# NorESMhub/BLOM

Measured on AMD Instinct MI355X. Metric: simulated-days/sec, higher is better.
Workload: dtype f64; 1 GPU; channel 208x512x53 as 1 tile(s) of 208x512x53 along i, 1 tile per GPU, isopyc_bulkml/remap/geopotential/uc/enscon, ntr=3 (TKE, length-scale slot, ideal age: the reference default build), baclin=900s batrop=18s lstep=50; config 2's step (phy/mod_blom_step.F90:96-253: init_fluxes, tmsmt1, cmnfld2, difest_isobml [the whole routine: diffusivities estimated every step (NorESM defaults incl. rhsctp; the; physics=full, forcing=default, spinup_steps=0

## Files before the change

### blom_amd/csrc/api.hip

```cpp
#include "../../include/blomgpu.h"
#include "blomgpu_internal.h"
#include "pow_libm.h"
#include "sin_libm.h"
#include "atan2_libm.h"
#include <algorithm>
#include <cstring>
#include <string_view>

static thread_local std::string g_err;

int ctx_fail(blomgpu_ctx *c, const std::string &msg) {
  if (c) c->err = msg;
  g_err = msg;
  return 1;
}

void ctx_drop_graphs(blomgpu_ctx *c) {
  for (auto &g : c->step_graph)
    if (g) { (void)hipGraphExecDestroy(g); g = nullptr; }
  c->steps_warm = 0;
}

void ctx_sync_view(blomgpu_ctx *c) {
  if (!c->dirty) return;
// ... 200 lines not shown
  {"mlrttp", O_STR, IN_C(mlrttp), 0},
  {"mommth", O_STR, IN_P(mommth), DIRTY, nullptr, nullptr, " mommth = ", {{"enscon", 0}, {"enecon", 1}, {"enedis", 2}}},
  {"pgfmth", O_STR, IN_P(pgfmth), DIRTY, nullptr, nullptr, " pgfmth = ", {{"geopotential", 0}, {"dynamic enthalpy", 1}}},
  {"advmth", O_STR, IN_P(advmth), DIRTY, nullptr, nullptr, " advmth = ", {{"remap", 0}, {"cppm", 1}}},
  {"bmcmth", O_STR, IN_P(bmcmth), DIRTY, nullptr, nullptr, " bmcmth = ", {{"uc", 0}, {"dluc", 1}}},
  {"eitmth", O_STR, IN_P(eitmth), DIRTY, nullptr, nullptr, " eitmth = ", {{"intdif", 1}, {"gm", 2}}},
  {"cppm_compatibility", O_STR, IN_C(cppm_compat), 0, nullptr, nullptr, " init_cppm: cppm_compatibility = ", {{"full", 1}, {"partial", 2}}},
  {"cppm_limiting", O_STR, IN_C(cppm_limiting), 0, nullptr, nullptr, " init_cppm: cppm_limiting = ", {{"monotonic", 1}, {"non_oscillatory", 2}}},
  {"mlrmth", O_STR, IN_C(mlrmth), 0, nullptr, nullptr, " init_eddtra: mlrmth = ", {{"none", 0}, {"fox08", 1}, {"bod23", 2}}},
  {"vcoord_type", O_STR, IN_P(vcoord_tag), DIRTY, nullptr, nullptr, " readnml_vcoord: vcoord_type = ",
   {{"isopyc_bulkml", 1}, {"cntiso_hybrid", 2}, {"plevel", 3}}},
  {"ale_reconstruction_method", O_STR, IN_C(ale_method), 0, nullptr, nullptr, " readnml_ale_regrid_remap: reconstruction_method = ",
   {{"plm", 101}, {"ppm", 102}, {"pqm", 103}}},
  {"ale_regrid_method", O_STR, IN_C(ale_regrid_method), 0, nullptr, nullptr, " readnml_ale_regrid_remap: regrid_method = ", {{"direct", 1}, {"nudge", 2}}},
  {"ale_density_limiting", O_STR, nullptr, 0, nullptr, nullptr, " readnml_ale_regrid_remap: density_limiting = ", {{"monotonic", 0}}},
  {"ale_tracer_limiting", O_STR, IN_C(ale_tracer_limiting), ALE_RESET, nullptr, nullptr, " readnml_ale_regrid_remap: tracer_limiting = ",
   {{"monotonic", 201}, {"non_oscillatory", 203}}},
  {"ale_velocity_limiting", O_STR, IN_C(ale_velocity_limiting), ALE_RESET, nullptr, nullptr, " readnml_ale_regrid_remap: velocity_limiting = ",
   {{"monotonic", 201}, {"non_oscillatory", 203}}},
};
static const Opt g_cesm_opts[] = {
  CB(smtfrc), CB(use_stream_relaxation), CI(nstep_in_cpl), CI(l1ci), CI(l2ci), CI(nstep_in_day), CI(nday_of_year), CI(cesm_single_sums),
};
static const Opt g_stepend_opts[] = {
  CB(step_time), CB(chkvar), CI(jwtype), {"chlopt", O_STR, IN_C(chlopt), 0},
  {"swamth", O_STR, IN_C(swamth), 0, nullptr, nullptr, " iniswa: swamth = ",
   {{"top-layer", SWA_TOP_LAYER}, {"jerlov", SWA_JERLOV}, {"chlorophyll_ma94", SWA_MA94}, {"chlorophyll_ohl03", SWA_OHL03}, {"spatial_frac_attlen", SWA_SPATIAL}}},
  {"sprfac", O_BOOL, IN_C(sprfac), 0, nullptr, [](blomgpu_ctx *c) { (void)stepend_set_sprfac(c); }},
  {"prfac", O_REAL, IN_C(prfac), READABLE},
};
static const Opt g_budget_opts[] = {
  CI(budget_step),
};
#undef IN_P
#undef IN_C
#undef PR
#undef PRR
#undef PI
#undef CR
#undef CI
#undef CB
#undef ONE_OR_TWO
#undef LMI
#undef RLX
static const Opt *find_opt(std::string_view name, unsigned kinds) {
  for (const Opt &o : g_opts)
    if (name == o.name && (kinds >> o.kind & 1)) return &o;
  for (const Opt &o : g_cesm_opts)
    if (name == o.name && (kinds >> o.kind & 1)) return &o;
  for (const Opt &o : g_stepend_opts)
    if (name == o.name && (kinds >> o.kind & 1)) return &o;
  for (const Opt &o : g_budget_opts)
    if (name == o.name && (kinds >> o.kind & 1)) return &o;
  return nullptr;
}
static int opt_lookup(blomgpu_ctx *c, const char *who, const char *name, unsigned kinds, const Opt **o) {
  if (!c || !name) return ctx_fail(c, std::string(who) + ": null argument");
  *o = find_opt(name, kinds);
  if (!*o || !((*o)->flags & KEEP_GRAPHS)) ctx_drop_graphs(c);
  return *o ? 0 : ctx_fail(c, std::string(who) + ": unknown option " + name);
}
static int set_number(blomgpu_ctx *c, const char *who, const char *name, unsigned kinds, double v) {
  const Opt *o;
  if (int rc = opt_lookup(c, who, name, kinds, &o)) return rc;
  if (o->kind == O_BOOL) v = v != 0;
  if (o->check)
    if (const char *refusal = o->check(v)) return ctx_fail(c, refusal);
  o->at(c).put(v);
  if (o->flags & DIRTY) c->dirty = true;
  if (o->after) o->after(c);
  return o->flags & ALE_RESET ? ale_reset(c) : 0;
}

template <class Launch>
static int libm_probe(blomgpu_ctx *c, int n, const double *a, const double *b, double *z, const char *who, Launch launch) {
  if (n <= 0) return 0;
  double *d = nullptr;
  HIPCHK(c, hipMalloc((void **)&d, sizeof(double) * 3 * (size_t)n));
  int rc = 0;
  if (hipMemcpyAsync(d, a, sizeof(double) * n, hipMemcpyHostToDevice, c->stream) != hipSuccess) rc = 1;
  if (b && hipMemcpyAsync(d + n, b, sizeof(double) * n, hipMemcpyHostToDevice, c->stream) != hipSuccess) rc = 1;
  launch(dim3((n + 255) / 256), d, d + n, d + 2 * (size_t)n);
  if (hipMemcpyAsync(z, d + 2 * (size_t)n, sizeof(double) * n, hipMemcpyDeviceToHost, c->stream) != hipSuccess) rc = 1;
  if (hipStreamSynchronize(c->stream) != hipSuccess) rc = 1;
  (void)hipFree(d);
// ... 137 lines not shown
  if (c->side) HIPCHK(c, hipStreamSynchronize(c->side));
  return 0;
}

int blomgpu_set_real(blomgpu_ctx *c, const char *name, double v) { return set_number(c, "blomgpu_set_real", name, 1u << O_REAL, v); }
int blomgpu_set_int(blomgpu_ctx *c, const char *name, int v) { return set_number(c, "blomgpu_set_int", name, 1u << O_INT | 1u << O_BOOL, v); }

int blomgpu_set_str(blomgpu_ctx *c, const char *name, const char *val) {
  const Opt *o = nullptr;
  const int rc = opt_lookup(c, "blomgpu_set_str", name, 1u << O_STR, &o);
  if (c) c->dirty = true;
  if (rc) return rc;
  if (!val) return ctx_fail(c, "blomgpu_set_str: null argument");
  const std::string v(val);
  if (!o->words[0].word) { *o->at(c).s = v; return 0; }
  for (const auto &w : o->words)
    if (w.word && v == w.word) {
      if (o->at) o->at(c).put(w.code);
      if (o->at && o->at(c).i == &c->swamth) c->swa_ready = false;
      return o->flags & ALE_RESET ? ale_reset(c) : 0;
    }
  return ctx_fail(c, o->refuse + v + " is unsupported!");
}

int blomgpu_get_real(blomgpu_ctx *c, const char *name, double *v) {
  const std::string s(name);
  if (const Opt *o = find_opt(s, 1u << O_REAL))
    if (o->flags & READABLE) { *v = *o->at(c).d; return 0; }
  if (s == "barotp_block_mode") { *v = bt_block_mode(c); return 0; }
  if (s == "barotp_shape") { *v = bt_shape_code(c); return 0; }
  if (s == "graph_steps") { *v = c->graph_steps; return 0; }
  if (s == "graph_failures") { *v = c->graph_failures; return 0; }
  if (s == "flux_diag_steps_skipped") { *v = (double)c->flux_diag_skipped; return 0; }
  if (s == "thermf_cesm_launches") { *v = (double)c->cesm_launches; return 0; }
  if (s == "thermf_ben02_launches") { *v = c->ben02_declared ? (double)c->cesm_launches : 0.; return 0; }
  if (c->step_time) {
    if (s == "xmi") { *v = c->xmi; return 0; }
    if (s == "nday_of_year") { *v = c->nday_of_year; return 0; }
    if (s.size() == 4 && s[0] == 'l' && s[1] >= '1' && s[1] <= '5' && s.compare(2, 2, "mi") == 0) { *v = c->lmi[s[1] - '1']; return 0; }
  }
  if (s == "sflxc") {
    if (!frc_declared(c)) return ctx_fail(c, "blomgpu_get_real: sflxc exists once blomgpu_inifrc_cesm has been called");
    double sum = 0.;
    HIPCHK(c, hipMemcpyAsync(&sum, c->cesm_sums, sizeof(double), hipMemcpyDeviceToHost, c->stream));
    HIPCHK(c, hipStreamSynchronize(c->stream));
    *v = sum / c->area;
    return 0;
  }
  if (s == "mxlayr_maxitr_entrain" || s == "mxlayr_maxitr_detrain") {
    *v = 0.;
    if (!c->err_dev) return 0;
    const int w = s == "mxlayr_maxitr_detrain" ? 5 : 6;
    int n = 0;
    HIPCHK(c, hipStreamSynchronize(c->stream));
    HIPCHK(c, hipMemcpy(&n, c->err_dev + w, sizeof(int), hipMemcpyDeviceToHost));
    HIPCHK(c, hipMemset(c->err_dev + w, 0, sizeof(int)));
    *v = n;
    return 0;
  }
  return ctx_fail(c, "blomgpu_get_real: unknown option " + s);
}

int blomgpu_option_name(int index, char *buf, int cap, int *kind) {
  if (index < 0 || index >= (int)(sizeof(g_opts) / sizeof(g_opts[0])) || !buf || cap < 2) return 1;
  snprintf(buf, cap, "%s", g_opts[index].name);
  if (kind) *kind = g_opts[index].kind;
// ... 432 lines not shown
    if (int rc = bud(1)) return rc;
    if (ale) {
      for (const StageId st : seq_ale) {
        if (c->tmsmt1_done_ahead && st == S_tmsmt1) { c->tmsmt1_done_ahead = false; continue; }
        if (c->eddtra_frozen && st == S_eddtra) continue;
        if (frc && st == S_pgforc)
          if (int rc = stage(S_sfcstr)) return rc;
        if (int rc = stage(st)) return rc;
        if (const int ncall = st == S_ale_regrid_remap ? 2 : st == S_diffus ? 3 : st == S_ale_vdiffm ? 4 : st == S_updtrc ? 5 : st == S_pbcor2 ? 6 : st == S_tmsmt2 ? 7 : 0)
          if (int rc = bud(ncall)) return rc;
        if (cesm && st == S_init_fluxes)
          if (int rc = stage(S_getfrc_cesm)) return rc;
        if (swa && st == S_init_fluxes)
          if (int rc = stage(S_updswa)) return rc;
        if (frc && st == S_momtum)
          if (int rc = stage(S_thermf)) return rc;
      }
    } else for (const StageId st : seq) {
      StageId run = c->live_slopes && st == S_halo_cmnfld2 ? S_cmnfld2 : st;
      if (c->full_physics && st == S_halo_difest) run = c->difest_live ? S_difest_isobml : S_difest_isobml_pre;
      if (c->full_physics && st == S_mxlayr_tail) {
        if (int rc = stage(S_thermf)) return rc;
        run = S_mxlayr;
      }
      if (c->eddtra_frozen && st == S_eddtra) continue;
      if (c->tmsmt1_done_ahead && st == S_tmsmt1) { c->tmsmt1_done_ahead = false; continue; }
      if (c->seq.fluxes_lean) {
        bool allowed = false;
        for (const StageId ok : {S_tmsmt1, S_halo_cmnfld2, S_cmnfld2, S_halo_difest, S_difest_isobml, S_difest_isobml_pre, S_eddtra, S_advect})
          allowed = allowed || run == ok;
        if (!allowed)
          return ctx_fail(c, std::string("blomgpu_step: stage ") + g_stages[run].name + " between the lean init_fluxes and advect: the flux arrays of level m are not zeroed (set lean_fluxes = 0)");
      }
      if ((c->seq.diapfl_mom_on_side && run != S_mxlayr) || (c->seq.updtrc_on_side && st == S_pbcor2)) {
        const int ev = c->seq.diapfl_mom_on_side ? 7 : 9;
        c->seq.diapfl_mom_on_side = c->seq.updtrc_on_side = false;
        if (ctx_side_done(c, ev) || ctx_side_join(c, ev)) return 1;
      }
      if (frc && st == S_pgforc)
        if (int rc = stage(S_sfcstr)) return rc;
      if (int rc = stage(run)) return rc;
      if (const int ncall = st == S_diffus ? 2 : st == S_convec ? 3 : st == S_diapfl ? 4 : st == S_updtrc ? 5 : st == S_pbcor2 ? 6 : st == S_tmsmt2 ? 7 : 0) {
        if (ncall == 5 && budget_on(c) && c->seq.updtrc_on_side) {
          c->seq.updtrc_on_side = false;
          if (ctx_side_done(c, 9) || ctx_side_join(c, 9)) return 1;
        }
        if (int rc = bud(ncall)) return rc;
      }
      if (cesm && st == S_init_fluxes)
        if (int rc = stage(S_getfrc_cesm)) return rc;
      if (swa && st == S_init_fluxes)
        if (int rc = stage(S_updswa)) return rc;
      if (st == S_halo_difest && c->seq.cmn_on_side) {
        c->seq.cmn_on_side = false;
        if (ctx_side_done(c, 4) || ctx_side_join(c, 4)) return 1;
      }
      static const StageId early_at[] = {S_halo_difest, S_eddtra, S_advect, S_pbcor1, S_diffus};
      if (st == early_at[c->mom_early_at < 0 || c->mom_early_at > 4 ? 0 : c->mom_early_at])
        if (int rc = st_momtum_early(c, m, n, mm, nn)) return rc;
    }
    leave.failed = false;
  }
  if (!ale && (c->cmnfld1 || c->full_physics))
    if (int rc = stage(S_cmnfld1)) return rc;
  if (dia_active(c))
    if (int rc = st_diaacc(ALL6)) return rc;
// ... 145 lines not shown
```

### blom_amd/csrc/blomgpu_internal.h

```cpp
#pragma once
#include <hip/hip_runtime.h>
#include <cstdint>
#include <string>
#include <unordered_map>
#include <vector>
#include "exp_libm.h"
#include "constants.h"
#include "workspace_slots.h"

#define NBDY 4

#ifdef BLOM_HOSTEMU
#define WAIT_VMCNT0() ((void)0)
#else
#define WAIT_VMCNT0() asm volatile("s_waitcnt vmcnt(0)" ::: "memory")
#endif

#define BLOM_REAL_FIELDS(X)                                                              \
                                                                          \
  X(u, 2 * K) X(v, 2 * K) X(dp, 2 * K) X(dpu, 2 * K) X(dpv, 2 * K) X(temp, 2 * K)        \
  X(saln, 2 * K) X(sigma, 2 * K) X(uflx, 2 * K) X(vflx, 2 * K) X(utflx, 2 * K)           \
  X(vtflx, 2 * K) X(usflx, 2 * K) X(vsflx, 2 * K)                                        \
  X(p, K + 1) X(pu, K + 1) X(pv, K + 1) X(phi, K + 1) X(cau, K) X(cav, K)                \
  X(ubflxs, 3) X(vbflxs, 3) X(ub, 2) X(vb, 2) X(pb, 2) X(pbu, 2) X(pbv, 2)               \
// ... 206 lines not shown
struct BtGlobal;
struct DiaState;
struct BudgetState;
struct TileTable {
  int npx = 0, npy = 0, itdm = 0, nranks = 0;
  std::vector<int> i0, ii;
  std::vector<int> j0, jj;
  std::vector<int> rank;
  void ew_neighbours(int px, int py, bool periodic, int *west, int *east) const;
  bool tensor_product() const;
};
const char *tiletable_build(int npx, int npy, int itdm, int jtdm, const int *i0_pe, const int *ii_pe, const int *j0_pe,
                            const int *jj_pe, TileTable *out);
struct Tiling {
  int npx = 1, npy = 1;
  int px = 0, py = 0;
  const TileTable *tab = nullptr;
  TileGroup *group = nullptr;
  RcclComm *rccl = nullptr;
  bool multi() const { return npx * npy > 1 || rccl != nullptr; }
};

struct StepState {
  bool in_sequence = false;
  bool defer_checks = false;
  bool remap_handed_over = false;
  bool pbcor1_handed_over = false;
  bool pbcor2_handed_over = false;
  bool pbcor2_dp_in_wk = false;
  bool fluxes_lean = false;
  bool fluxes_zeroed = false;
  bool mom_early_done = false;
  bool convec_col_ahead = false;
  bool cmn_on_side = false;
  bool diapfl_mom_on_side = false, updtrc_on_side = false;
  bool pscan_done_ahead = false;
};

struct BtShape { int ti, tj, pair_pref; bool persist, block; };
constexpr int BT_NSHAPES = 7;
constexpr BtShape kBtShapes[BT_NSHAPES] = {{32, 16, 4, false, false}, {32, 8, 2, false, false}, {16, 8, 1, false, false},
                                           {26, 16, 3, true, true},   {26, 15, 0, true, true},  {40, 16, 5, true, false},
                                           {40, 15, 0, true, false}};

struct blomgpu_ctx {
  std::string expcnf = "channel";
  bool csdiag = false;
  int cnsvdi = 0;
  int cppm_compat = 1;
  int cppm_limiting = 2;
  int ale_method = 102, ale_upper_bndr_ord = 6, ale_lower_bndr_ord = 4, ale_tracer_limiting = 203, ale_velocity_limiting = 203;
  bool ale_tracer_pc_upper = true, ale_tracer_pc_lower = false, ale_velocity_pc_upper = true, ale_velocity_pc_lower = false;
  bool ale_density_pc_upper = false, ale_density_pc_lower = false;
  int ale_regrid_method = 2, ale_k_range_plevel = 1;
  double ale_regrid_nudge_ts = 86400., ale_stab_fac_limit = .75, ale_dpvar_fac = .75, ale_smooth_diff_max = 50000.;
  int ale_dktzu = 4, ale_dktzl = 2;
  double ale_dpmin_interior = .1 * ONEM;
  int ndiff_rec_per_face = 0;
  int ndiff_surface_align = 1;
  double rm0 = 1.2, rm5 = 0., niwgf = 0., niwbf = .35, niwlf = .5;
  std::string mlrttp = "constant";
  double trxday = 0., srxday = 0., trxdpt = 1., srxdpt = 1., trxlim = 1.5, srxlim = .5, sref = 34.65, area = 0., xmi = 0.;
  int lmi[5] = {11, 12, 1, 2, 3};
  bool aptflx = false, apsflx = false, ditflx = false, disflx = false, srxbal = false;
  int ntda = 0;
  double swamxd = 200., brine_mlbase_frac = 0.;
// ... 15 lines not shown
  int check_period = 8;
  bool timing = false;
  int use_graph = 0;
  int overlap = 1;
  int phys_dag = 7;
  int mom_early_at = 0;
  int lean_fluxes = 1;
  int tmsmt_fold = 1;
  int tmsmt_ahead = 1;
  int remap_fold = 0;
  int remap_nfirst = 4;
  int halo_overlap = 1;
  int barotp_fused = 1;
  int barotp_tile = 0;
  int barotp_persist = 1;
  int barotp_block = 1;
  int barotp_overlap = 0;
  int barotp_rimbuf = 1;
  int barotp_arctic_persist = 1;
  int barotp_arctic_fused = 1;
  int arctic_strips = 0;
  int pgf_uv_pair = 0;
  int pgf_uv_ring = 7;
  int pgf_reuse = 0;
  int pgf_copy_fused = 1;
  int scan_reassoc = 0;
  int mom_aw_split = 0;
  int mom_force_aw = 0;
  int momtum_order = 0;
  int momtum_lds_pad = 0;
  int momtum_bs = 0;
  int momtum_chunks_a = 0, momtum_chunks_b = 0;
  int convec_nsingle = 2;
  int cmn_nslope_nb = 4;
  int diapfl_du = 8;
  int diffus_shfl = 0;
  int kprof_sel = 1;

  DevView h;
  DevView *d = nullptr;
  bool dirty = true;
  int device = 0;
  hipStream_t stream = nullptr;
  bool stream_borrowed = false;
  hipStream_t xstream = nullptr, halo_stream = nullptr;
  hipEvent_t ev_fork = nullptr, ev_join = nullptr;
  hipStream_t side = nullptr;
  hipEvent_t ev_side[10] = {};
  DevView hv[4];
  DevView *dv[4] = {nullptr, nullptr, nullptr, nullptr};
  double *wk_mom = nullptr, *p_alt = nullptr, *pu_alt = nullptr, *pv_alt = nullptr;
  hipStream_t side3 = nullptr;
  hipEvent_t ev_side3[2] = {nullptr, nullptr};
  int mom_aw_key = -1, mom_aw_n[2] = {0, 0};
  int *mom_aw_dev = nullptr;
  int nlev_real[NF_REAL];
  int nlev_int[NF_INT];
  std::unordered_map<std::string, int> real_ids, int_ids;
  std::unordered_map<std::string, KTimer> timers;
  Tiling tiling;
  BtGlobal *bt_global = nullptr;
  std::string err;
  int *err_dev = nullptr;
  StepState seq;
  bool tmsmt1_ahead = false, tmsmt1_done_ahead = false;
  bool flux_diag = true, keep_flux_diag = false;
  long long flux_diag_skipped = 0;
  hipGraphExec_t step_graph[2] = {nullptr, nullptr};
  int steps_done = 0;
  int steps_warm = 0;
  long long graph_steps = 0;
  int graph_failures = 0;
  bool cppm_ready = false;
  void *ale = nullptr;
  double *ale_plevel = nullptr;
  bool bt_restart = true;
  unsigned bt_epoch = 0;
  unsigned *bt_flags = nullptr;
  int bt_flags_words = 0;
  int num_cus = 0;
  int bt_blocks_per_cu[BT_NSHAPES][2] = {{-1, -1}, {-1, -1}, {-1, -1}, {-1, -1}, {-1, -1}, {-1, -1}, {-1, -1}};
  long long *bt_prof = nullptr;
  long long *kprof = nullptr;
  int kprof_words = 0;
  double *arc_strip = nullptr;
  size_t arc_cap = 0;
  double *xcsum_dev = nullptr;
  double *xcsum_buf = nullptr;
  double budget[5][7][2] = {};
  int budget_step = 0;
  BudgetState *bud = nullptr;
  DiaState *dia = nullptr;
  std::vector<double> dia_edges;
  std::vector<double> dia_sigdia;
  bool cesm_declared = false;
  int nflxdi[48] = {};
  long long cesm_launches = 0;
  double *cesm_sums = nullptr, *cesm_rows = nullptr;
  bool ben02_declared = false;
// ... 21 lines not shown
static inline bool flux_diag_on(const blomgpu_ctx *c) { return !c->seq.in_sequence || c->flux_diag; }

int  ctx_fail(blomgpu_ctx *c, const std::string &msg);
int  ctx_pack_masks(blomgpu_ctx *c);
void ctx_sync_view(blomgpu_ctx *c);
void ctx_drop_graphs(blomgpu_ctx *c);
#define HIPCHK(c, call)                                                                   \
  do {                                                                                    \
    hipError_t e_ = (call);                                                               \
    if (e_ != hipSuccess)                                                                 \
      return ctx_fail((c), std::string(#call) + ": " + hipGetErrorString(e_));            \
  } while (0)

struct TimeScope {
  blomgpu_ctx *c;
  hipEvent_t a = nullptr, b = nullptr;
  const char *what;
  hipStream_t st = nullptr;
  TimeScope(blomgpu_ctx *c_, const char *w, hipStream_t s = nullptr);
  ~TimeScope();
};

int st_init_fluxes(blomgpu_ctx *, int m, int n, int mm, int nn, int k1m, int k1n);
int st_tmsmt1(blomgpu_ctx *, int nn);
int st_tmsmt2(blomgpu_ctx *, int m, int mm, int nn, int k1m);
int st_initms(blomgpu_ctx *, int mm);
int st_advect(blomgpu_ctx *, int m, int n, int mm, int nn, int k1m, int k1n);
int st_pbcor1(blomgpu_ctx *, int m, int n, int mm, int nn, int k1m, int k1n);
int st_pbcor2(blomgpu_ctx *, int m, int n, int mm, int nn, int k1m, int k1n);
int st_diffus(blomgpu_ctx *, int m, int n, int mm, int nn, int k1m, int k1n);
int st_pgforc(blomgpu_ctx *, int m, int n, int mm, int nn, int k1m, int k1n);
int st_momtum(blomgpu_ctx *, int m, int n, int mm, int nn, int k1m, int k1n);
int st_momtum_fused_layers(blomgpu_ctx *, int m, int n, int mm, int nn, int part);
int st_momtum_early(blomgpu_ctx *, int m, int n, int mm, int nn);
int st_convec_column_ahead(blomgpu_ctx *, int n, int nn);
int st_diapfl(blomgpu_ctx *, int n, int nn, int k1n);
int st_convec(blomgpu_ctx *, int m, int n, int mm, int nn, int k1m, int k1n);
int st_updtrc(blomgpu_ctx *, int m, int n, int mm, int nn, int k1m, int k1n);
int st_xcsum(blomgpu_ctx *, const double *a, int itype, double *sum);
int st_xcsum_dev(blomgpu_ctx *, const double *a, int itype, int slot, double **sums_dev);
int st_thermf(blomgpu_ctx *, int m, int n, int mm, int nn, int k1m, int k1n);
int cesm_inifrc(blomgpu_ctx *);
int cesm_field(blomgpu_ctx *, int fid);
void cesm_free(blomgpu_ctx *);
static inline bool cesm_on(const blomgpu_ctx *c) { return c->cesm_declared && c->expcnf == "cesm"; }
int frc_alloc(blomgpu_ctx *, double **p, int nlev);
int frc_sum_buffers(blomgpu_ctx *);
int st_getfrc_cesm(blomgpu_ctx *);
int st_sfcstr_cesm(blomgpu_ctx *);
int st_thermf_cesm(blomgpu_ctx *, int m, int n, int mm, int nn, int k1m, int k1n);
static inline bool ben02_expcnf(const std::string &e) { return e == "ben02clim" || e == "ben02syn" || e == "single_column"; }
static inline bool ben02_on(const blomgpu_ctx *c) { return c->ben02_declared && ben02_expcnf(c->expcnf); }
static inline bool frc_declared(const blomgpu_ctx *c) { return c->cesm_declared || c->ben02_declared; }
int ben02_inifrc(blomgpu_ctx *);
int ben02_reset_tda(blomgpu_ctx *);
void ben02_free(blomgpu_ctx *);
int st_sfcstr_ben02(blomgpu_ctx *);
int st_thermf_ben02(blomgpu_ctx *, int m, int n, int mm, int nn, int k1m, int k1n);
enum { SWA_NONE = 0, SWA_TOP_LAYER, SWA_JERLOV, SWA_MA94, SWA_OHL03, SWA_SPATIAL };
static inline bool swa_chlorophyll(const blomgpu_ctx *c) { return c->swamth == SWA_MA94 || c->swamth == SWA_OHL03; }
int stepend_iniswa(blomgpu_ctx *);
int stepend_set_sprfac(blomgpu_ctx *);
int stepend_step_time(blomgpu_ctx *, int ns1);
int stepend_step_check(blomgpu_ctx *);
int stepend_check_errors(blomgpu_ctx *);
void stepend_free(blomgpu_ctx *);
// ... 190 lines not shown
```

### blom_amd/csrc/stage_convec.hip

```cpp
#include "blomgpu_internal.h"
#include "eos.h"
#include "diapfl_common.h"

#define MAXTR 64

__global__ __launch_bounds__(64) void k_convec_column(const DevView *__restrict__ Vp, int n, int nn, int *errflag) {
  const DevView &V = *Vp;
  THREAD_IJ_XCD(V);
  if (j < 1 || j > V.jj || i < 1 || i > V.ii || !V.m[I_ip][c]) return;
  const int kk = V.kk, ntr = V.ntr;
  const size_t np = V.nplane;
  gd_t ttem = V.f[F_temp] + c + (size_t)nn * np - np, ssal = V.f[F_saln] + c + (size_t)nn * np - np;
  gd_t delp = V.f[F_dp] + c + (size_t)nn * np - np, dens = V.f[F_sigma] + c + (size_t)nn * np - np;
  gcd_t densr = V.f[F_sigmar] + c - np;
  gd_t trc = V.f[F_trc] + c + (size_t)nn * np - np;
  const size_t ntl = (size_t)2 * kk * np;
#define TT(k) ttem[(size_t)(k) * np]
#define SS(k) ssal[(size_t)(k) * np]
#define DP(k) delp[(size_t)(k) * np]
#define DN(k) dens[(size_t)(k) * np]
#define DR(k) densr[(size_t)(k) * np]
#define TR(nt, k) trc[(size_t)(nt) * ntl + (size_t)(k) * np]
  double tdps, sdps, dps, ttmp, stmp, dtmp, q = 0.;

// ... 367 lines not shown
  switch (c->convec_nsingle) {
    case -1: hipLaunchKernelGGL(k_convec_velocity_flat, plane_grid(c->h, 2, 64), dim3(64), 0, c->stream, c->d, nn); break;
    case 0: hipLaunchKernelGGL(k_convec_velocity<0>, plane_grid(c->h, 2, 64), dim3(64), 0, c->stream, c->d, nn); break;
    case 1: hipLaunchKernelGGL(k_convec_velocity<1>, plane_grid(c->h, 2, 64), dim3(64), 0, c->stream, c->d, nn); break;
    case 2: hipLaunchKernelGGL(k_convec_velocity<2>, plane_grid(c->h, 2, 64), dim3(64), 0, c->stream, c->d, nn); break;
    case 3: hipLaunchKernelGGL(k_convec_velocity<3>, plane_grid(c->h, 2, 64), dim3(64), 0, c->stream, c->d, nn); break;
    default: hipLaunchKernelGGL(k_convec_velocity<1000>, plane_grid(c->h, 2, 64), dim3(64), 0, c->stream, c->d, nn); break;
  }
  HIPCHK(c, hipGetLastError());
  return 0;
}

int st_convec_column_ahead(blomgpu_ctx *c, int n, int nn) {
  const DevView &h = c->h;
  c->seq.convec_col_ahead = false;
  if (h.ntr > MAXTR || h.P.vcoord_tag != 1) return 0;
  if (int rc = ctx_err_words(c)) return rc;
  if (int rc = ctx_side_fork(c, 2)) return rc;
  hipLaunchKernelGGL(k_convec_column, plane_grid(h, 1, 64), dim3(64), 0, c->side, c->d, n, nn, c->err_dev + 3);
  HIPCHK(c, hipGetLastError());
  if (int rc = ctx_side_done(c, 3)) return rc;
  c->seq.convec_col_ahead = true;
  return 0;
}

int st_convec(blomgpu_ctx *c, int m, int n, int mm, int nn, int k1m, int k1n) {
  (void)m; (void)mm; (void)k1m; (void)k1n;
  const DevView &h = c->h;
  if (h.ntr > MAXTR) return ctx_fail(c, "convec: too many tracers for the device kernels");
  if (h.P.vcoord_tag != 1) return ctx_fail(c, "convec is only called for isopyc_bulkml (phy/mod_blom_step.F90:172-176)");
  if (int rc = ctx_err_words(c)) return rc;
  {
    TimeScope ts(c, "convec");
    if (c->seq.convec_col_ahead) {
      c->seq.convec_col_ahead = false;
      if (int rc = ctx_side_join(c, 3)) return rc;
    } else
      hipLaunchKernelGGL(k_convec_column, plane_grid(h, 1, 64), dim3(64), 0, c->stream, c->d, n, nn, c->err_dev + 3);
    if (int rc = st_xctilr(c, h.f[F_p], 1, h.kk + 1, 1, 1, 1)) return rc;
    if (int rc = st_convec_velocity(c, nn)) return rc;
    hipLaunchKernelGGL(k_convec_dpudpv, plane_grid(h, h.kk), dim3(256), 0, c->stream, c->d, nn);
  }
  HIPCHK(c, hipGetLastError());
  return 0;
}
```

### blom_amd/csrc/stage_momtum.hip

```cpp
#include "blomgpu_internal.h"

#include "momtum_common.h"


__global__ void k_mom_pupv(const DevView *__restrict__ Vp, int off, int lo, int hi, int ring) {
  const DevView &V = *Vp;
  THREAD_IJ_XCD(V);
  if (j < lo || j > V.jj + hi || i < lo || i > V.ii + hi) return;
  if (ring && j >= 1 && j <= V.jj && i >= 1 && i <= V.ii) return;
  const size_t np = V.nplane;
  if (V.m[I_iu][c]) column_scan(V.f[F_pu][c], V.f[F_dpu] + (size_t)off * np + c, V.f[F_pu] + c, np, V.kk);
  if (V.m[I_iv][c]) column_scan(V.f[F_pv][c], V.f[F_dpv] + (size_t)off * np + c, V.f[F_pv] + c, np, V.kk);
}

__global__ void k_mom_pscan(const DevView *__restrict__ Vp, int off, int lo, int hi, int ring) {
  const DevView &V = *Vp;
  THREAD_IJ_XCD(V);
  if (j < lo || j > V.jj + hi || i < lo || i > V.ii + hi || !V.m[I_ip][c]) return;
  if (ring && j >= 1 && j <= V.jj && i >= 1 && i <= V.ii) return;
  const size_t np = V.nplane;
  column_scan(V.f[F_p][c], V.f[F_dp] + (size_t)off * np + c, V.f[F_p] + c, np, V.kk);
}

__global__ void k_mom_drag(const DevView *__restrict__ Vp, int n, int nn) {
// ... 43 lines not shown
    q[c + np] = V.f[F_vbflxs_p][c + om] * tsfac / (V.f[F_pbv][c + om] * sx);
    q[c + 3 * np] = V.f[F_vbflxs_p][c + on] * tsfac / (V.f[F_pbv][c + on] * sx);
  }
}

int st_mom_pupv(blomgpu_ctx *c, int off, int lo, int hi) {
  hipLaunchKernelGGL(k_mom_pupv, plane_grid(c->h, 1, 64), dim3(64), 0, c->stream, c->d, off, lo, hi, 0);
  HIPCHK(c, hipGetLastError());
  return 0;
}

static int momtum_visc_chain(blomgpu_ctx *c, int m, int n, int mm, int nn) {
  const DevView &h = c->h;
  hipLaunchKernelGGL(k_mom_pupv, plane_grid(h, 1, 64), dim3(64), 0, c->stream, ctx_view(c, VIEW_MOM_A), mm, -1, 2, 0);
  hipLaunchKernelGGL(k_mom_qplanes, plane_grid(h, 1, 256), dim3(256), 0, c->stream, ctx_view(c, VIEW_MOM_A), m, n);
  return st_momtum_fused_layers(c, m, n, mm, nn, 1);
}

int st_momtum_early(blomgpu_ctx *c, int m, int n, int mm, int nn) {
  c->seq.mom_early_done = false;
  if (!ctx_overlap_on(c) || c->tiling.multi()) return 0;
  if (int rc = st_xctilr(c, c->h.f[F_difwgt], 1, 1, 2, 2, 1)) return rc;
  if (int rc = ctx_side_fork(c, 0)) return rc;
  hipStream_t main = c->stream;
  c->stream = c->side;
  const int rc = momtum_visc_chain(c, m, n, mm, nn);
  c->stream = main;
  if (rc) return rc;
  if (int rc2 = ctx_side_done(c, 1)) return rc2;
  c->seq.mom_early_done = true;
  return 0;
}

int st_momtum(blomgpu_ctx *c, int m, int n, int mm, int nn, int k1m, int k1n) {
  (void)k1m; (void)k1n;
  const DevView &h = c->h;
  const dim3 gcol = plane_grid(h, 1, 64), b64(64);
  if (ctx_overlap_on(c) && !c->tiling.multi())
    if (int rc = st_convec_column_ahead(c, n, nn)) return rc;
  TimeScope ts(c, "momtum");
  hipLaunchKernelGGL(k_mom_pscan, gcol, b64, 0, c->stream, ctx_view(c, VIEW_MOM_B), mm, -1, 2, 0);
  hipLaunchKernelGGL(k_mom_pscan, gcol, b64, 0, c->stream, c->d, mm, -1, 2, c->seq.in_sequence && h.P.vcoord_tag == 1 ? 1 : 0);
  hipLaunchKernelGGL(k_mom_pupv, gcol, b64, 0, c->stream, c->d, mm, -1, 2, 1);
  hipLaunchKernelGGL(k_mom_drag, gcol, b64, 0, c->stream, ctx_view(c, VIEW_MOM_B), n, nn);
  if (c->seq.mom_early_done) {
    c->seq.mom_early_done = false;
    if (int rc = ctx_side_join(c, 1)) return rc;
  } else {
    if (int rc = st_xctilr(c, h.f[F_difwgt], 1, 1, 2, 2, 1)) return rc;
    if (int rc = momtum_visc_chain(c, m, n, mm, nn)) return rc;
  }
  return st_momtum_fused_layers(c, m, n, mm, nn, 2);
}
```

### blom_amd/csrc/stage_momtum_fused.hip

```cpp
#include "momtum_common.h"
#include <type_traits>

#define WK2V(w) ((gcd_t) * (double *const volatile CONST_AS *)&Vp->wk2d + (size_t)(w) * np)

#define GLOBAL_AS BLOM_GAS
#define GF(V, id) ((gcd_t)(V).f[id])

__device__ inline void march_item(int kk, int jj, int nchunk_, int nstrip, int &k, int &ja, int &jb, int &strip, const int *list = nullptr) {
  const bool chunk_major = nchunk_ < 0;
  const int nchunk = chunk_major ? -nchunk_ : nchunk_;
  const unsigned nitem = gridDim.x, lin = blockIdx.x;
  const unsigned xq = lin & 7u, sq = lin >> 3, q = nitem >> 3, rr = nitem & 7u;
  unsigned item = xq * q + (xq < rr ? xq : rr) + sq;
  if (list) {
    const int e = list[item / kk];
    k = item % kk;
    strip = e % nstrip;
    const int ch = e / nstrip, rows = (jj + nchunk - 1) / nchunk;
    ja = 1 + ch * rows;
    jb = ja + rows - 1 < jj ? ja + rows - 1 : jj;
    return;
  }
  strip = item % nstrip;
  item /= nstrip;
// ... 618 lines not shown
        un = fmax2(-umax, fmin2(umax, un + ub)) - ub;
        un_[(size_t)k * np] = un;
        uabove = un;
        tot = tot + un * dn;
      }
    }
  }
  tot = tot / (isv ? V.f[F_pbv_p] : V.f[F_pbu_p])[c];
  double pacc = (isv ? V.f[F_pv] : V.f[F_pu])[c];
  gd_t pun = (isv ? V.f[F_pv] : V.f[F_pu]) + c;
  for (int k0 = 0; k0 < kk; k0 += COLUMN_U) {
    double a[COLUMN_U], b[COLUMN_U], d[COLUMN_U], e[COLUMN_U], f[COLUMN_U];
#pragma unroll
    for (int u = 0; u < COLUMN_U; u++) {
      const size_t o = (size_t)(k0 + u < kk ? k0 + u : kk - 1) * np;
      a[u] = dpum[o]; b[u] = dpun[o]; d[u] = un_[o]; e[u] = sm[o]; f[u] = dpuold[o];
    }
#pragma unroll
    for (int u = 0; u < COLUMN_U; u++) {
      const int k = k0 + u;
      if (k < kk) {
        const double dn = b[u];
        const double un = d[u] - tot;
        un_[(size_t)k * np] = un;
        um[(size_t)k * np] = (e[u] + un * wuv2 * dn) / (wuv1 * a[u] + ONEMM + wuv2 * (f[u] + dn));
        pacc = pacc + dn;
        pun[(size_t)(k + 1) * np] = pacc;
      }
    }
  }
  (isv ? V.f[F_vtotn] : V.f[F_utotn])[c] = tot * (1. / V.P.delt1);
}

template <int BS>
__global__ __launch_bounds__(64) void k_mom_classify(const DevView *__restrict__ Vp, int nchunk, int nstrip, int *flags) {
  const DevView &V = *Vp;
  const int l = threadIdx.x, ni = V.ni, ii = V.ii, jj = V.jj;
  const int e = blockIdx.x, strip = e % nstrip, ch = e / nstrip;
  const int rows = (jj + nchunk - 1) / nchunk, ja = 1 + ch * rows, jb = ja + rows - 1 < jj ? ja + rows - 1 : jj;
  constexpr int HL = 4, HR = 4, OW = BS - HL - HR;
  const int ox0 = NBDY + strip * OW;
  bool all = ja <= jb && ox0 <= ii + NBDY - 1;
  for (int l0 = 0; l0 < BS; l0 += 64) {
    const int x = ox0 - HL + l0 + l;
    const int xl = x < 2 ? 2 : (x > ni - 3 ? ni - 3 : x);
    for (int r = ja - 6; r <= jb + 4; r++) {
      const int rc = r < -2 ? -2 : (r > jj + 3 ? jj + 3 : r);
      if ((V.m[I_mpack][xl + ni * (rc + NBDY - 1)] & 15) != 15) all = false;
    }
  }
  all = WAVE_ALL(all);
  if (l == 0) flags[e] = all ? 1 : 0;
}

static int mom_aw_lists(blomgpu_ctx *c, int BS, int nca, int nsa, const int **la_, int *na, const int **lb_, int *nb) {
  const int key = BS * 100000 + nca * 100 + nsa;
  if (c->mom_aw_key != key) {
    hipStreamCaptureStatus cs = hipStreamCaptureStatusNone;
    if (hipStreamIsCapturing(c->stream, &cs) != hipSuccess || cs != hipStreamCaptureStatusNone) return 1;
    if (c->mom_aw_dev) { (void)hipFree(c->mom_aw_dev); c->mom_aw_dev = nullptr; }
    const int n = nca * nsa;
    int *flags = nullptr;
    HIPCHK(c, hipMalloc((void **)&flags, sizeof(int) * n));
    ctx_sync_view(c);
    if (BS == 64) hipLaunchKernelGGL(k_mom_classify<64>, dim3(n), dim3(64), 0, c->stream, c->d, nca, nsa, flags);
    else if (BS == 128) hipLaunchKernelGGL(k_mom_classify<128>, dim3(n), dim3(64), 0, c->stream, c->d, nca, nsa, flags);
    else hipLaunchKernelGGL(k_mom_classify<256>, dim3(n), dim3(64), 0, c->stream, c->d, nca, nsa, flags);
    std::vector<int> hf(n), lists;
    HIPCHK(c, hipMemcpyAsync(hf.data(), flags, sizeof(int) * n, hipMemcpyDeviceToHost, c->stream));
    HIPCHK(c, hipStreamSynchronize(c->stream));
    (void)hipFree(flags);
    for (int e = 0; e < n; e++) if (hf[e]) lists.push_back(e);
    c->mom_aw_n[0] = (int)lists.size();
    for (int e = 0; e < n; e++) if (!hf[e]) lists.push_back(e);
    c->mom_aw_n[1] = n - c->mom_aw_n[0];
    HIPCHK(c, hipMalloc((void **)&c->mom_aw_dev, sizeof(int) * (n > 0 ? n : 1)));
    HIPCHK(c, hipMemcpy(c->mom_aw_dev, lists.data(), sizeof(int) * n, hipMemcpyHostToDevice));
    c->mom_aw_key = key;
  }
  *la_ = c->mom_aw_dev; *na = c->mom_aw_n[0];
  *lb_ = c->mom_aw_dev + c->mom_aw_n[0]; *nb = c->mom_aw_n[1];
  return 0;
}

template <int BS>
static void launch_marches(blomgpu_ctx *c, int m, int n, int mm, int nn, int nca, int ncb, int part) {
  const DevView &h = c->h;
  const int nsa = (h.ii + (BS - 8) - 1) / (BS - 8), nsb = (h.ii + (BS - 4) - 1) / (BS - 4);
  const size_t la = sizeof(double) * 37 * (BS + 4) + c->momtum_lds_pad, lb = sizeof(double) * (h.P.mommth == 2 ? 35 : 21) * (BS + 4) + c->momtum_lds_pad;
  (void)hipFuncSetAttribute((const void *)k_mom_visc_march<BS, 2>, hipFuncAttributeMaxDynamicSharedMemorySize, (int)la);
  (void)hipFuncSetAttribute((const void *)k_mom_cor_march<BS, true>, hipFuncAttributeMaxDynamicSharedMemorySize, (int)lb);
  (void)hipFuncSetAttribute((const void *)k_mom_cor_march<BS, false>, hipFuncAttributeMaxDynamicSharedMemorySize, (int)lb);
  if (part != 2) {
    TimeScope tk(c, "k_mom_visc_march");
    (void)hipFuncSetAttribute((const void *)k_mom_visc_march<BS, 1>, hipFuncAttributeMaxDynamicSharedMemorySize, (int)la);
    const int *l_aw = nullptr, *l_mx = nullptr;
    int n_aw = 0, n_mx = 0;
    const bool split = c->mom_aw_split && h.P.allwet && !c->mom_force_aw && !c->momtum_order && mom_aw_lists(c, BS, nca, nsa, &l_aw, &n_aw, &l_mx, &n_mx) == 0;
    if (c->mom_force_aw)
      hipLaunchKernelGGL((k_mom_visc_march<BS, 1>), dim3(h.kk * nca * nsa), dim3(BS), la, c->stream, ctx_view(c, VIEW_MOM_A), m, n, mm, nn, c->momtum_order ? nca : -nca, nsa, (const int *)nullptr);
    else if (split) {
      const bool third = n_aw && n_mx && c->mom_aw_split == 2;
      if (third) {
        if (!c->side3) {
          if (hipStreamCreateWithFlags(&c->side3, hipStreamNonBlocking) != hipSuccess) c->side3 = nullptr;
          for (auto &e : c->ev_side3) if (hipEventCreateWithFlags(&e, hipEventDisableTiming) != hipSuccess) e = nullptr;
        }
      }
      if (third && c->side3 && c->ev_side3[0] && c->ev_side3[1]) {
        (void)hipEventRecord(c->ev_side3[0], c->stream);
        (void)hipStreamWaitEvent(c->side3, c->ev_side3[0], 0);
        hipLaunchKernelGGL((k_mom_visc_march<BS, 2>), dim3(h.kk * n_mx), dim3(BS), la, c->side3, ctx_view(c, VIEW_MOM_A), m, n, mm, nn, -nca, nsa, l_mx);
        hipLaunchKernelGGL((k_mom_visc_march<BS, 1>), dim3(h.kk * n_aw), dim3(BS), la, c->stream, ctx_view(c, VIEW_MOM_A), m, n, mm, nn, -nca, nsa, l_aw);
        (void)hipEventRecord(c->ev_side3[1], c->side3);
        (void)hipStreamWaitEvent(c->stream, c->ev_side3[1], 0);
      } else {
        if (n_mx) hipLaunchKernelGGL((k_mom_visc_march<BS, 2>), dim3(h.kk * n_mx), dim3(BS), la, c->stream, ctx_view(c, VIEW_MOM_A), m, n, mm, nn, -nca, nsa, l_mx);
        if (n_aw) hipLaunchKernelGGL((k_mom_visc_march<BS, 1>), dim3(h.kk * n_aw), dim3(BS), la, c->stream, ctx_view(c, VIEW_MOM_A), m, n, mm, nn, -nca, nsa, l_aw);
      }
    } else
      hipLaunchKernelGGL((k_mom_visc_march<BS, 2>), dim3(h.kk * nca * nsa), dim3(BS), la, c->stream, ctx_view(c, VIEW_MOM_A), m, n, mm, nn, c->momtum_order ? nca : -nca, nsa, (const int *)nullptr);
  }
  if (part == 1) return;
  TimeScope tk(c, "k_mom_cor_march");
  if (h.P.mommth == 2)
    hipLaunchKernelGGL((k_mom_cor_march<BS, true>), dim3(h.kk * ncb * nsb), dim3(BS), lb, c->stream, ctx_view(c, VIEW_MOM_B), m, n, mm, nn, c->momtum_order ? ncb : -ncb, nsb);
  else
    hipLaunchKernelGGL((k_mom_cor_march<BS, false>), dim3(h.kk * ncb * nsb), dim3(BS), lb, c->stream, ctx_view(c, VIEW_MOM_B), m, n, mm, nn, c->momtum_order ? ncb : -ncb, nsb);
}

int st_momtum_fused_layers(blomgpu_ctx *c, int m, int n, int mm, int nn, int part) {
  const DevView &h = c->h;
  const int cus = c->num_cus > 0 ? c->num_cus : 256;
  const int bs = c->momtum_bs > 0 ? c->momtum_bs : 64;
  auto chunks = [&](int slots, int nstrip, int opt) {
    int nc = opt > 0 ? opt : slots / (h.kk * nstrip);
    if (nc > (h.jj + 15) / 16) nc = (h.jj + 15) / 16;
    return nc < 1 ? 1 : nc;
  };
  const int nsa = (h.ii + (bs - 8) - 1) / (bs - 8), nsb = (h.ii + (bs - 4) - 1) / (bs - 4);
  const int nca = chunks(cus * (bs == 64 ? 8 : 160 * 1024 / (37 * (bs + 4) * 8)), nsa, c->momtum_chunks_a);
  const int ncb = chunks(cus * 8 * 64 / bs, nsb, c->momtum_chunks_b);
  if (bs == 64) launch_marches<64>(c, m, n, mm, nn, nca, ncb, part);
  else if (bs == 128) launch_marches<128>(c, m, n, mm, nn, nca, ncb, part);
  else if (bs == 256) launch_marches<256>(c, m, n, mm, nn, nca, ncb, part);
  else return ctx_fail(c, "momtum: momtum_bs must be 64, 128 or 256");
  if (part != 1) hipLaunchKernelGGL(k_mom_column_from, plane_grid(h, 2, 64), dim3(64), 0, c->stream, ctx_view(c, VIEW_MOM_C), m, mm, nn);
  HIPCHK(c, hipGetLastError());
  return 0;
}
```

Measured before the change: 1.655 simulated-days/sec.

## Fold convec velocity remap into momtum's final column kernel

After: 1.664 simulated-days/sec, median of 6. No clear change (+0.5%).

```diff
diff --git a/blom_amd/csrc/api.hip b/blom_amd/csrc/api.hip
--- a/blom_amd/csrc/api.hip
+++ b/blom_amd/csrc/api.hip
@@ -256,6 +256,9 @@
 static const Opt g_budget_opts[] = {
   CI(budget_step),
 };
+static const Opt g_handover_opts[] = {
+  CI(mom_convec_fold),
+};
 #undef IN_P
 #undef IN_C
 #undef PR
@@ -275,6 +278,8 @@
   for (const Opt &o : g_stepend_opts)
     if (name == o.name && (kinds >> o.kind & 1)) return &o;
   for (const Opt &o : g_budget_opts)
+    if (name == o.name && (kinds >> o.kind & 1)) return &o;
+  for (const Opt &o : g_handover_opts)
     if (name == o.name && (kinds >> o.kind & 1)) return &o;
   return nullptr;
 }
@@ -478,6 +483,8 @@
   if (s == "graph_steps") { *v = c->graph_steps; return 0; }
   if (s == "graph_failures") { *v = c->graph_failures; return 0; }
   if (s == "flux_diag_steps_skipped") { *v = (double)c->flux_diag_skipped; return 0; }
+  if (s == "mom_convec_folds") { *v = (double)c->mom_convec_folds; return 0; }
+  if (s == "convec_vel_launches") { *v = (double)c->convec_vel_launches; return 0; }
   if (s == "thermf_cesm_launches") { *v = (double)c->cesm_launches; return 0; }
   if (s == "thermf_ben02_launches") { *v = c->ben02_declared ? (double)c->cesm_launches : 0.; return 0; }
   if (c->step_time) {
@@ -976,6 +983,8 @@
         if (!allowed)
           return ctx_fail(c, std::string("blomgpu_step: stage ") + g_stages[run].name + " between the lean init_fluxes and advect: the flux arrays of level m are not zeroed (set lean_fluxes = 0)");
       }
+      if (c->seq.convec_vel_folded && run != S_convec)
+        return ctx_fail(c, std::string("blomgpu_step: stage ") + g_stages[run].name + " behind a momtum that has handed its velocity columns to convec: dpu, dpv are not the new layers' yet (set mom_convec_fold = 0)");
       if ((c->seq.diapfl_mom_on_side && run != S_mxlayr) || (c->seq.updtrc_on_side && st == S_pbcor2)) {
         const int ev = c->seq.diapfl_mom_on_side ? 7 : 9;
         c->seq.diapfl_mom_on_side = c->seq.updtrc_on_side = false;
diff --git a/blom_amd/csrc/blomgpu_internal.h b/blom_amd/csrc/blomgpu_internal.h
--- a/blom_amd/csrc/blomgpu_internal.h
+++ b/blom_amd/csrc/blomgpu_internal.h
@@ -262,6 +262,7 @@
   bool fluxes_zeroed = false;
   bool mom_early_done = false;
   bool convec_col_ahead = false;
+  bool convec_vel_folded = false;
   bool cmn_on_side = false;
   bool diapfl_mom_on_side = false, updtrc_on_side = false;
   bool pscan_done_ahead = false;
@@ -343,6 +344,7 @@
   int momtum_bs = 0;
   int momtum_chunks_a = 0, momtum_chunks_b = 0;
   int convec_nsingle = 2;
+  int mom_convec_fold = 1;
   int cmn_nslope_nb = 4;
   int diapfl_du = 8;
   int diffus_shfl = 0;
@@ -376,6 +378,7 @@
   StepState seq;
   bool tmsmt1_ahead = false, tmsmt1_done_ahead = false;
   bool flux_diag = true, keep_flux_diag = false;
+  long long mom_convec_folds = 0, convec_vel_launches = 0;
   long long flux_diag_skipped = 0;
   hipGraphExec_t step_graph[2] = {nullptr, nullptr};
   int steps_done = 0;
@@ -463,6 +466,9 @@
 int st_pgforc(blomgpu_ctx *, int m, int n, int mm, int nn, int k1m, int k1n);
 int st_momtum(blomgpu_ctx *, int m, int n, int mm, int nn, int k1m, int k1n);
 int st_momtum_fused_layers(blomgpu_ctx *, int m, int n, int mm, int nn, int part);
+int st_momtum_column_convec(blomgpu_ctx *, int m, int mm, int nn);
+bool mom_convec_fold_applies(const blomgpu_ctx *);
+int st_convec_front(blomgpu_ctx *, int n, int nn);
 int st_momtum_early(blomgpu_ctx *, int m, int n, int mm, int nn);
 int st_convec_column_ahead(blomgpu_ctx *, int n, int nn);
 int st_diapfl(blomgpu_ctx *, int n, int nn, int k1n);
diff --git a/blom_amd/csrc/stage_convec.hip b/blom_amd/csrc/stage_convec.hip
--- a/blom_amd/csrc/stage_convec.hip
+++ b/blom_amd/csrc/stage_convec.hip
@@ -423,15 +423,30 @@
   if (int rc = ctx_err_words(c)) return rc;
   {
     TimeScope ts(c, "convec");
-    if (c->seq.convec_col_ahead) {
-      c->seq.convec_col_ahead = false;
-      if (int rc = ctx_side_join(c, 3)) return rc;
-    } else
-      hipLaunchKernelGGL(k_convec_column, plane_grid(h, 1, 64), dim3(64), 0, c->stream, c->d, n, nn, c->err_dev + 3);
-    if (int rc = st_xctilr(c, h.f[F_p], 1, h.kk + 1, 1, 1, 1)) return rc;
-    if (int rc = st_convec_velocity(c, nn)) return rc;
+    const bool folded = c->seq.convec_vel_folded;
+    c->seq.convec_vel_folded = false;
+    if (!folded) {
+      if (int rc = st_convec_front(c, n, nn)) return rc;
+      if (int rc = st_convec_velocity(c, nn)) return rc;
+      c->convec_vel_launches++;
+    }
     hipLaunchKernelGGL(k_convec_dpudpv, plane_grid(h, h.kk), dim3(256), 0, c->stream, c->d, nn);
   }
   HIPCHK(c, hipGetLastError());
   return 0;
 }
+
+bool mom_convec_fold_applies(const blomgpu_ctx *c) {
+  return c->mom_convec_fold && c->seq.in_sequence && c->h.P.vcoord_tag == 1 && !c->tiling.multi() && c->h.ntr <= MAXTR;
+}
+
+int st_convec_front(blomgpu_ctx *c, int n, int nn) {
+  const DevView &h = c->h;
+  if (int rc = ctx_err_words(c)) return rc;
+  if (c->seq.convec_col_ahead) {
+    c->seq.convec_col_ahead = false;
+    if (int rc = ctx_side_join(c, 3)) return rc;
+  } else
+    hipLaunchKernelGGL(k_convec_column, plane_grid(h, 1, 64), dim3(64), 0, c->stream, c->d, n, nn, c->err_dev + 3);
+  return st_xctilr(c, h.f[F_p], 1, h.kk + 1, 1, 1, 1);
+}
diff --git a/blom_amd/csrc/stage_momtum.hip b/blom_amd/csrc/stage_momtum.hip
--- a/blom_amd/csrc/stage_momtum.hip
+++ b/blom_amd/csrc/stage_momtum.hip
@@ -99,13 +99,9 @@
   return 0;
 }
 
-int st_momtum(blomgpu_ctx *c, int m, int n, int mm, int nn, int k1m, int k1n) {
-  (void)k1m; (void)k1n;
+static int st_momtum_front(blomgpu_ctx *c, int m, int n, int mm, int nn) {
   const DevView &h = c->h;
   const dim3 gcol = plane_grid(h, 1, 64), b64(64);
-  if (ctx_overlap_on(c) && !c->tiling.multi())
-    if (int rc = st_convec_column_ahead(c, n, nn)) return rc;
-  TimeScope ts(c, "momtum");
   hipLaunchKernelGGL(k_mom_pscan, gcol, b64, 0, c->stream, ctx_view(c, VIEW_MOM_B), mm, -1, 2, 0);
   hipLaunchKernelGGL(k_mom_pscan, gcol, b64, 0, c->stream, c->d, mm, -1, 2, c->seq.in_sequence && h.P.vcoord_tag == 1 ? 1 : 0);
   hipLaunchKernelGGL(k_mom_pupv, gcol, b64, 0, c->stream, c->d, mm, -1, 2, 1);
@@ -117,5 +113,29 @@
     if (int rc = st_xctilr(c, h.f[F_difwgt], 1, 1, 2, 2, 1)) return rc;
     if (int rc = momtum_visc_chain(c, m, n, mm, nn)) return rc;
   }
+  return 0;
+}
+
+int st_momtum(blomgpu_ctx *c, int m, int n, int mm, int nn, int k1m, int k1n) {
+  (void)k1m; (void)k1n;
+  if (ctx_overlap_on(c) && !c->tiling.multi())
+    if (int rc = st_convec_column_ahead(c, n, nn)) return rc;
+  if (mom_convec_fold_applies(c)) {
+    {
+      TimeScope ts(c, "momtum");
+      if (int rc = st_momtum_front(c, m, n, mm, nn)) return rc;
+      if (int rc = st_momtum_fused_layers(c, m, n, mm, nn, 3)) return rc;
+    }
+    {
+      TimeScope ts(c, "convec");
+      if (int rc = st_convec_front(c, n, nn)) return rc;
+    }
+    TimeScope ts(c, "momtum");
+    if (int rc = st_momtum_column_convec(c, m, mm, nn)) return rc;
+    c->seq.convec_vel_folded = true;
+    return 0;
+  }
+  TimeScope ts(c, "momtum");
+  if (int rc = st_momtum_front(c, m, n, mm, nn)) return rc;
   return st_momtum_fused_layers(c, m, n, mm, nn, 2);
 }
diff --git a/blom_amd/csrc/stage_momtum_fused.hip b/blom_amd/csrc/stage_momtum_fused.hip
--- a/blom_amd/csrc/stage_momtum_fused.hip
+++ b/blom_amd/csrc/stage_momtum_fused.hip
@@ -674,6 +674,144 @@
   (isv ? V.f[F_vtotn] : V.f[F_utotn])[c] = tot * (1. / V.P.delt1);
 }
 
+#define MC_U 4
+#define MC_L 4
+__global__ __launch_bounds__(64) __attribute__((amdgpu_waves_per_eu(4, 4))) void k_mom_column_convec(const DevView *__restrict__ Vp, int m, int mm, int nn KPROF_ARGS) {
+  const DevView &V = *Vp;
+  unsigned bx_, by_;
+  xcd_block(bx_, by_);
+  const int t_ = bx_ * blockDim.x + threadIdx.x;
+  if (t_ >= V.nplane) return;
+  const int i = t_ % V.ni - (NBDY - 1), j = t_ / V.ni - (NBDY - 1);
+  const size_t c = t_;
+  if (j < 1 || j > V.jj || i < 1 || i > V.ii) return;
+  const bool isv = by_ == 1;
+  if (!(isv ? V.m[I_iv][c] : V.m[I_iu][c])) return;
+  [[maybe_unused]] const int wid = (int)(by_ * gridDim.x + bx_);
+  KPROF_MARK(wid, 0);
+  const size_t np = V.nplane;
+  const int kk = V.kk;
+  gd_t u = isv ? V.f[F_v] : V.f[F_u];
+  gcd_t sm = WK(V, isv ? MF_VM : MF_UM);
+  gd_t sn = WK(V, isv ? MF_VN : MF_UN);
+  gcd_t dpu = isv ? V.f[F_dpv] : V.f[F_dpu], dpuold = isv ? V.f[F_dpvold] : V.f[F_dpuold];
+  const double umax = (isv ? V.f[F_vmax] : V.f[F_umax])[c];
+  const double ub = (isv ? V.f[F_vb] : V.f[F_ub])[c + (size_t)(m - 1) * np];
+  const double wuv1 = V.P.wuv1, wuv2 = V.P.wuv2;
+  double tot = 0., uabove = 0.;
+  const double *dpum = dpu + c + (size_t)mm * np, *dpun = dpu + c + (size_t)nn * np;
+  double *um = u + c + (size_t)mm * np, *unew = u + c + (size_t)nn * np - np;
+  gd_t pun = (isv ? V.f[F_pv] : V.f[F_pu]) + c;
+  sm += c; sn += c; dpuold += c;
+  gcd_t pc = V.f[F_p] + c, pw = V.f[F_p] + (isv ? c - V.ni : c - 1);
+  double q0[MC_L], q1[MC_L];
+  int knq = 1;
+#pragma unroll
+  for (int b = 0; b < MC_L; b++) {
+    const size_t o = (size_t)(knq + b <= kk ? knq + b : kk) * np;
+    q0[b] = pc[o]; q1[b] = pw[o];
+  }
+  const double pu0 = pun[0];
+  double pbot = pu0;
+  for (int k0 = 0; k0 < kk; k0 += COLUMN_U) {
+    double a[COLUMN_U], b[COLUMN_U], d[COLUMN_U];
+#pragma unroll
+    for (int u = 0; u < COLUMN_U; u++) {
+      const size_t o = (size_t)(k0 + u < kk ? k0 + u : kk - 1) * np;
+      a[u] = dpum[o]; b[u] = dpun[o]; d[u] = sn[o];
+    }
+#pragma unroll
+    for (int u = 0; u < COLUMN_U; u++) {
+      const int k = k0 + u;
+      if (k < kk) {
+        const double dn = b[u];
+        const double q = fmin2(fmin2(a[u], dn), ONEM);
+        double un = d[u];
+        const double ukan = k == 0 ? un : uabove;
+        un = (un * q + ukan * (ONEM - q)) / ONEM;
+        un = fmax2(-umax, fmin2(umax, un + ub)) - ub;
+        sn[(size_t)k * np] = un;
+        uabove = un;
+        tot = tot + un * dn;
+        pbot = pbot + dn;
+      }
+    }
+  }
+  KPROF_MARK(wid, 1);
+  tot = tot / (isv ? V.f[F_pbv_p] : V.f[F_pbu_p])[c];
+  double pacc = pu0;
+  int kn = 1, ia = MC_L, ktail = kk + 1;
+  double pn[MC_L] = {};
+  double pn_lo = 0., udpn = 0., po_lo = 0.;
+  auto merge = [&](const double v, const double po_hi, const bool last) {
+    while (kn <= kk) {
+      if (ia == MC_L) {
+#pragma unroll
+        for (int b = 0; b < MC_L; b++) pn[b] = .5 * (fmin2(pbot, q0[b]) + fmin2(pbot, q1[b]));
+        ia = 0;
+        knq += MC_L;
+#pragma unroll
+        for (int b = 0; b < MC_L; b++) {
+          const size_t o = (size_t)(knq + b <= kk ? knq + b : kk) * np;
+          q0[b] = pc[o]; q1[b] = pw[o];
+        }
+      }
+      const double pn_hi = ia == 0 ? pn[0] : ia == 1 ? pn[1] : ia == 2 ? pn[2] : pn[3];
+      static_assert(MC_L == 4, "the selection above names MC_L entries");
+      double r = 0.;
+      if (pn_hi - pn_lo == 0.) {
+      } else if (!last && pn_hi > po_hi) {
+        udpn = udpn + v * (po_hi - fmax2(po_lo, pn_lo));
+        break;
+      } else
+        r = (udpn + v * (pn_hi - fmax2(po_lo, pn_lo))) / (pn_hi - pn_lo);
+      unew[(size_t)kn * np] = r;
+      pn_lo = pn_hi;
+      udpn = 0.;
+      kn = kn + 1;
+      ia = ia + 1;
+      if (pn_lo == pbot) { ktail = kn; kn = kk + 1; }
+    }
+    po_lo = po_hi;
+  };
+  double ulast = 0.;
+  for (int k0 = 0; k0 < kk; k0 += MC_U) {
+    double a[MC_U], b[MC_U], d[MC_U], e[MC_U], f[MC_U];
+#pragma unroll
+    for (int u = 0; u < MC_U; u++) {
+      const size_t o = (size_t)(k0 + u < kk ? k0 + u : kk - 1) * np;
+      a[u] = dpum[o]; b[u] = dpun[o]; d[u] = sn[o]; e[u] = sm[o]; f[u] = dpuold[o];
+    }
+#pragma unroll
+    for (int u = 0; u < MC_U; u++) {
+      const int k = k0 + u;
+      if (k < kk) {
+        const double dn = b[u];
+        const double un = d[u] - tot;
+        um[(size_t)k * np] = (e[u] + un * wuv2 * dn) / (wuv1 * a[u] + ONEMM + wuv2 * (f[u] + dn));
+        pacc = pacc + dn;
+        pun[(size_t)(k + 1) * np] = pacc;
+        merge(un, pacc, false);
+        ulast = un;
+      }
+    }
+  }
+  merge(ulast, 1.e300, true);
+  KPROF_MARK(wid, 2);
+  for (int k = 1; k <= kk; k++)
+    if (k >= ktail) unew[(size_t)k * np] = 0.;
+  (isv ? V.f[F_vtotn] : V.f[F_utotn])[c] = tot * (1. / V.P.delt1);
+  KPROF_MARK(wid, 3);
+}
+
+int st_momtum_column_convec(blomgpu_ctx *c, int m, int mm, int nn) {
+  TimeScope tk(c, "k_mom_column_convec");
+  hipLaunchKernelGGL(k_mom_column_convec, plane_grid(c->h, 2, 64), dim3(64), 0, c->stream, ctx_view(c, VIEW_MOM_C), m, mm, nn KPROF_PASS(6));
+  HIPCHK(c, hipGetLastError());
+  c->mom_convec_folds++;
+  return 0;
+}
+
 template <int BS>
 __global__ __launch_bounds__(64) void k_mom_classify(const DevView *__restrict__ Vp, int nchunk, int nstrip, int *flags) {
   const DevView &V = *Vp;
@@ -733,7 +871,7 @@
   (void)hipFuncSetAttribute((const void *)k_mom_visc_march<BS, 2>, hipFuncAttributeMaxDynamicSharedMemorySize, (int)la);
   (void)hipFuncSetAttribute((const void *)k_mom_cor_march<BS, true>, hipFuncAttributeMaxDynamicSharedMemorySize, (int)lb);
   (void)hipFuncSetAttribute((const void *)k_mom_cor_march<BS, false>, hipFuncAttributeMaxDynamicSharedMemorySize, (int)lb);
-  if (part != 2) {
+  if (part != 2 && part != 3) {
     TimeScope tk(c, "k_mom_visc_march");
     (void)hipFuncSetAttribute((const void *)k_mom_visc_march<BS, 1>, hipFuncAttributeMaxDynamicSharedMemorySize, (int)la);
     const int *l_aw = nullptr, *l_mx = nullptr;
@@ -787,7 +925,7 @@
   else if (bs == 128) launch_marches<128>(c, m, n, mm, nn, nca, ncb, part);
   else if (bs == 256) launch_marches<256>(c, m, n, mm, nn, nca, ncb, part);
   else return ctx_fail(c, "momtum: momtum_bs must be 64, 128 or 256");
-  if (part != 1) hipLaunchKernelGGL(k_mom_column_from, plane_grid(h, 2, 64), dim3(64), 0, c->stream, ctx_view(c, VIEW_MOM_C), m, mm, nn);
+  if (part != 1 && part != 3) hipLaunchKernelGGL(k_mom_column_from, plane_grid(h, 2, 64), dim3(64), 0, c->stream, ctx_view(c, VIEW_MOM_C), m, mm, nn);
   HIPCHK(c, hipGetLastError());
   return 0;
 }
```
